# tuneinsight/lattigo

Measured on AMD Instinct MI355X. Metric: ciphertext-mul+relin ops/s, higher is better.
Workload: dtype u64; 1 GPU; BGV logN=15, 12 Q-limbs [55,45x11] + 3 P-limbs [55x3], T=65537: ct x ct MulRelin (tensor + gadget product + ModDown), inputs resident in HBM; batch_per_gpu=256, logN=15, L=12, alpha=3, beta=4, parallelism=1 independent replicas, ciphertext-sharded

## Files before the change

lattigo_amd/csrc/kernels.hip:

```cpp
#include "kernels.h"

#include <atomic>
#include <cstdio>
#include <cstdlib>
#include <type_traits>
#include <mutex>
#include <unordered_map>
#include <vector>

namespace he {

namespace {
struct ProfRec { int id; hipEvent_t e0, e1; double bytes; };
struct ProfState { std::vector<ProfRec> recs; };
std::mutex g_prof_mu;
std::atomic<int> g_prof_active{0};
std::unordered_map<hipStream_t, ProfState> g_prof;
std::vector<hipEvent_t> g_prof_pool;
hipEvent_t prof_event_locked() {
    if (!g_prof_pool.empty()) { hipEvent_t e = g_prof_pool.back(); g_prof_pool.pop_back(); return e; }
    hipEvent_t e;
    (void)hipEventCreate(&e);
    return e;
}
// ... 1315 lines not shown
            const uint64_t qu = ldc(mcw, 0);
            uint64_t r0[16], r1[16], r2[16], r3[16];
            round0(xA);
            __syncthreads();
            rows_lds_xfer_f64<LOGB, 4>(xA, lds, tau, 0, LOGB - 4, true);
            if (AA.e.ext_f64) {
#pragma unroll
                for (int k = 0; k < 16; k++) xB[k] = __longlong_as_double((long long)wB[k]);
            } else {
#pragma unroll
                for (int k = 0; k < 16; k++) xB[k] = u52_to_f64(wB[k]);
            }
            round0(xB);
            __syncthreads();
            MAC_STAMP2(50);
            round1(xA, tau);
            __syncthreads();
            rows_lds_xfer_f64<LOGB, 4>(xB, lds, tau, 0, LOGB - 4, true);
            MAC_STAMP2(51);
            __builtin_amdgcn_sched_barrier(0);
            {
                const uint64_t *pa0 = AA.e.ta0 + meoff(AA.e, ME_TA0, AA.e.ta0_bs, cur.bz, AA.nbatch) + off;
                const uint64_t *pb0 = AA.e.tb0 + meoff(AA.e, ME_TB0, AA.e.tb0_bs, cur.bz, AA.nbatch) + off;
#pragma unroll
                for (int k = 0; k < 16; k++) { r0[k] = pa0[(unsigned)(k * T)]; r1[k] = pb0[(unsigned)(k * T)]; }
            }
            __builtin_amdgcn_sched_barrier(0);
            rows_round16_f64<false>(xA, t2, q, qi);
#pragma unroll
            for (int k = 0; k < 16; k++) xA[k] -= reduce_f64(acc0[k], q, qi);
            __syncthreads();
            MAC_STAMP2(52);
            round1(xB, tau);
            mac_final_xfer<LOGB>(xA, lds, tau, true);
            MAC_STAMP2(53);
            rows_round16_f64<false>(xB, t2, q, qi);
#pragma unroll
            for (int k = 0; k < 16; k++) xB[k] -= reduce_f64(acc1[k], q, qi);
            __builtin_amdgcn_sched_barrier(0);
            {
                const uint64_t *pa1 = AA.e.ta1 + meoff(AA.e, ME_TA1, AA.e.ta1_bs, cur.bz, AA.nbatch) + off;
                const uint64_t *pb1 = AA.e.tb1 + meoff(AA.e, ME_TB1, AA.e.tb1_bs, cur.bz, AA.nbatch) + off;
#pragma unroll
                for (int k = 0; k < 16; k++) { r2[k] = pa1[(unsigned)(k * T)]; r3[k] = pb1[(unsigned)(k * T)]; }
            }
            __builtin_amdgcn_sched_barrier(0);
            __syncthreads();
            MAC_STAMP2(54);
#pragma unroll
            for (int k = 0; k < 16; k++) xA[k] = lds[lds_phys(k * T + tau)];
            __syncthreads();
            mac_final_xfer<LOGB>(xB, lds, tau, true);
            MAC_STAMP2(55);
            auto cvtb = [&](uint64_t (&w)[16], double (&dd)[16]) {
                const uint64_t twoq_u = qu << 1, brc0 = ldc(mcw, 2);
                bool big = false;
#pragma unroll
                for (int k = 0; k < 16; k++) big = big || w[k] >= twoq_u;
                if (__any(big)) {
#pragma unroll
                    for (int k = 0; k < 16; k++) w[k] = bred_add_lazy(w[k], qu, brc0);
                }
#pragma unroll
                for (int k = 0; k < 16; k++) dd[k] = u52_to_f64(w[k]);
            };
            const double tsp = AA.e.tsp[cur.l];
            double u[16], v[16];
            cvtb(r0, u); cvtb(r1, v);
#pragma unroll
            for (int k = 0; k < 16; k++) {
                const double tt = modmul_f64(modmul_f64(u[k], v[k], q, qi), tsp, q, qi) + modmul_f64(xA[k], sp, q, qi);
                stnt(&op0[(unsigned)(k * T)], canon_f64(tt, q, qi));
            }
            __builtin_amdgcn_sched_barrier(0);
            __syncthreads();
            MAC_STAMP2(56);
#pragma unroll
            for (int k = 0; k < 16; k++) xB[k] = lds[lds_phys(k * T + tau)];
            double u2[16], v2[16];
            cvtb(r2, u2); cvtb(r3, v2);
#pragma unroll
            for (int k = 0; k < 16; k++) {
                const double wv = modmul_f64(u[k], v2[k], q, qi) + modmul_f64(u2[k], v[k], q, qi);
                const double tt = modmul_f64(wv, tsp, q, qi) + modmul_f64(xB[k], sp, q, qi);
                stnt(&op1[(unsigned)(k * T)], canon_f64(tt, q, qi));
            }
            MAC_STAMP2(57);
        } else if constexpr (EPI) {
            auto ext_pass = [&](auto cc) __attribute__((always_inline)) {
                const int c = cc;
                unsigned tau_d = threadIdx.x;
                asm volatile("" : "+v"(tau_d));
                const unsigned tau = tau_d, lane = tau & 63u;
                const double *pw = pbuf + wv * 1024u + lane;
                MAC_STAMP2(48 + c * 4 + 0);
                asm volatile("s_waitcnt vmcnt(0)" ::: "memory");
                double x[16];
                if (AA.e.ext_f64) {
#pragma unroll
                    for (int k = 0; k < 16; k++) x[k] = pw[k * 64];
                } else {
#pragma unroll
                    for (int k = 0; k < 16; k++) x[k] = u52_to_f64((uint64_t)__double_as_longlong(pw[k * 64]));
                }
                const uint64_t *nsrc = next_src(A.m.beta + c);
                const bool second = c != 0;
                const size_t off = (size_t)cur.out_limb * A.N + cur.rowoff + tau;
                uint64_t *op = (second ? AA.e.out1 + meoff(AA.e, ME_OUT1, AA.e.out1_bs, cur.bz, AA.nbatch) : AA.e.out0 + meoff(AA.e, ME_OUT0, AA.e.out0_bs, cur.bz, AA.nbatch)) + off;
                const double sp = AA.e.sp[cur.l];
                const uint64_t *mcw = reinterpret_cast<const uint64_t *>(A.mc + cur.mi);
                const uint64_t qu = ldc(mcw, 0);
                const bool tensor = LOGB == 13 && AA.e.tensor != 0;
                const bool addw = !tensor && (second ? AA.e.has_w1 : AA.e.has_w0) != 0;
                double kd0[16], kd1[16];
                MAC_STAMP2(48 + c * 4 + 1);
                constexpr bool prefetch = LOGB == 12;
                const uint64_t *pa0 = nullptr, *pa1 = nullptr, *pb0 = nullptr, *pb1 = nullptr, *wp = nullptr;
                if (tensor) {
                    pa0 = AA.e.ta0 + meoff(AA.e, ME_TA0, AA.e.ta0_bs, cur.bz, AA.nbatch) + off; pa1 = AA.e.ta1 + meoff(AA.e, ME_TA1, AA.e.ta1_bs, cur.bz, AA.nbatch) + off;
                    pb0 = AA.e.tb0 + meoff(AA.e, ME_TB0, AA.e.tb0_bs, cur.bz, AA.nbatch) + off; pb1 = AA.e.tb1 + meoff(AA.e, ME_TB1, AA.e.tb1_bs, cur.bz, AA.nbatch) + off;
                } else if (addw) {
                    wp = (second ? AA.e.w1 + meoff(AA.e, ME_W1, AA.e.w1_bs, cur.bz, AA.nbatch) : AA.e.w0 + meoff(AA.e, ME_W0, AA.e.w0_bs, cur.bz, AA.nbatch)) + off;
                }
                constexpr int NB = 4;
                uint64_t A0[NB], A1[NB], A2[NB], A3[NB];
                if constexpr (prefetch) transform(addw ? 1 : 0, x, tau, lane, nsrc, reinterpret_cast<const double *>(wp), nullptr, kd0, kd1);
                else transform(0, x, tau, lane, nsrc, nullptr, nullptr, kd0, kd1);
#pragma unroll
                for (int k = 0; k < 16; k++) x[k] -= reduce_f64(acc0[k], q, qi);
                mac_final_xfer<LOGB>(x, lds, tau, true);
                __syncthreads();
#pragma unroll
                for (int k = 0; k < 16; k++) x[k] = lds[lds_phys(k * T + tau)];
                MAC_STAMP2(48 + c * 4 + 2);
                if (tensor) {
                    const double tsp = AA.e.tsp[cur.l];
                    const uint64_t twoq_u = qu << 1, brc0 = ldc(mcw, 2);
                    auto cvtb = [&](uint64_t (&w)[NB], double (&dd)[NB]) {
                        bool big = false;
#pragma unroll
                        for (int k = 0; k < NB; k++) big = big || w[k] >= twoq_u;
                        if (__any(big)) {
#pragma unroll
                            for (int k = 0; k < NB; k++) w[k] = bred_add_lazy(w[k], qu, brc0);
                        }
#pragma unroll
                        for (int k = 0; k < NB; k++) dd[k] = u52_to_f64(w[k]);
                    };
                    auto issue = [&](auto hc, uint64_t (&r0)[NB], uint64_t (&r1)[NB], uint64_t (&r2)[NB], uint64_t (&r3)[NB]) {
                        constexpr int h = decltype(hc)::value;
#pragma unroll
                        for (int k = 0; k < NB; k++) { const unsigned e = (unsigned)((NB * h + k) * T); r0[k] = pa0[e]; r1[k] = pb0[e]; }
                        if (second) {
#pragma unroll
                            for (int k = 0; k < NB; k++) { const unsigned e = (unsigned)((NB * h + k) * T); r2[k] = pa1[e]; r3[k] = pb1[e]; }
                        }
                        __builtin_amdgcn_sched_barrier(0);
                    };
                    auto finish = [&](auto hc, uint64_t (&r0)[NB], uint64_t (&r1)[NB], uint64_t (&r2)[NB], uint64_t (&r3)[NB]) {
                        constexpr int h = decltype(hc)::value;
                        double u[NB], v[NB], u2[NB], v2[NB], wv[NB];
                        cvtb(r0, u); cvtb(r1, v);
                        if (second) {
                            cvtb(r2, u2); cvtb(r3, v2);
#pragma unroll
                            for (int k = 0; k < NB; k++) wv[k] = modmul_f64(u[k], v2[k], q, qi) + modmul_f64(u2[k], v[k], q, qi);
                        } else {
#pragma unroll
                            for (int k = 0; k < NB; k++) wv[k] = modmul_f64(u[k], v[k], q, qi);
                        }
#pragma unroll
                        for (int k = 0; k < NB; k++) {
                            const int i = NB * h + k;
                            const double tt = modmul_f64(wv[k], tsp, q, qi) + modmul_f64(x[i], sp, q, qi);
                            stnt(&op[(unsigned)(i * T)], canon_f64(tt, q, qi));
                        }
                        __builtin_amdgcn_sched_barrier(0);
                    };
#define HE_H(n) std::integral_constant<int, n>{}
                    issue(HE_H(0), A0, A1, A2, A3); finish(HE_H(0), A0, A1, A2, A3);
                    issue(HE_H(1), A0, A1, A2, A3); finish(HE_H(1), A0, A1, A2, A3);
                    issue(HE_H(2), A0, A1, A2, A3); finish(HE_H(2), A0, A1, A2, A3);
                    issue(HE_H(3), A0, A1, A2, A3); finish(HE_H(3), A0, A1, A2, A3);
#undef HE_H
                } else if (addw) {
                    uint64_t wv[16];
                    if constexpr (prefetch) {
#pragma unroll
                        for (int k = 0; k < 16; k++) wv[k] = (uint64_t)__double_as_longlong(kd0[k]);
                    } else {
#pragma unroll
                        for (int k = 0; k < 16; k++) wv[k] = ldnt(&wp[(unsigned)(k * T)]);
                    }
#pragma unroll
                    for (int k = 0; k < 16; k++) {
                        const uint64_t v = canon_f64(modmul_f64(x[k], sp, q, qi), q, qi);
                        uint64_t *dp = &op[(unsigned)(k * T)];
                        if constexpr (SCAT) dp = op - (cur.rowoff + tau) + auto_dest((unsigned)(cur.rowoff + tau) + (unsigned)(k * T), AA.e.sc_ginv, AA.e.sc_logN);
                        stnt(dp, cred(wv[k] + v, qu));
                    }
                } else {
#pragma unroll
                    for (int k = 0; k < 16; k++) {
                        uint64_t *dp = &op[(unsigned)(k * T)];
                        if constexpr (SCAT) dp = op - (cur.rowoff + tau) + auto_dest((unsigned)(cur.rowoff + tau) + (unsigned)(k * T), AA.e.sc_ginv, AA.e.sc_logN);
                        stnt(dp, canon_f64(modmul_f64(x[k], sp, q, qi), q, qi));
                    }
                }
                MAC_STAMP2(48 + c * 4 + 3);
#pragma unroll
                for (int k = 0; k < 16; k++) acc0[k] = acc1[k];
            };
            if constexpr (LOGB == 12) {
                ext_pass(std::integral_constant<int, 0>{});
                ext_pass(std::integral_constant<int, 1>{});
            } else {
#pragma unroll 1
                for (int c = 0; c < 2; c++) ext_pass(c);
            }
        }
        const int ol = cur.out_limb;
        uint64_t *o0 = nullptr, *o1 = nullptr;
        unsigned tau_t = threadIdx.x;
        asm volatile("" : "+v"(tau_t));
        const unsigned tau = tau_t;
        if constexpr (!EPI) {
            o0 = (cur.isP ? A.o0P + voff(A.oP0_tab, A.oP0_bs, cur.bz) : A.o0Q + voff(A.oQ0_tab, A.oQ0_bs, cur.bz)) + (size_t)ol * A.N + cur.rowoff + tau;
            o1 = (cur.isP ? A.o1P + voff(A.oP1_tab, A.oP1_bs, cur.bz) : A.o1Q + voff(A.oQ1_tab, A.oQ1_bs, cur.bz)) + (size_t)ol * A.N + cur.rowoff + tau;
        }
        [[maybe_unused]] uint64_t gs_av[16], gs_p0[16], gs_p1[16];
        [[maybe_unused]] const uint64_t *gs_ap = nullptr;
        if constexpr (!EPI && SCAT) {
            __builtin_amdgcn_sched_barrier(0);
            const size_t src = cur.rowoff + tau;
            if (AA.e.has_w0) gs_ap = (cur.isP ? AA.e.w1 + meoff(AA.e, ME_W1, AA.e.w1_bs, cur.bz, AA.nbatch) : AA.e.w0 + meoff(AA.e, ME_W0, AA.e.w0_bs, cur.bz, AA.nbatch)) + (size_t)ol * A.N + src;
            if (gs_ap) {
#pragma unroll
                for (int k = 0; k < 16; k++) gs_av[k] = ldnt(&gs_ap[(unsigned)(k * T)]);
            }
            if (AA.e.gs_accum) {
                const uint64_t *b0p = o0 - src;
#pragma unroll
                for (int k = 0; k < 16; k++) gs_p0[k] = b0p[auto_dest((unsigned)src + (unsigned)(k * T), AA.e.sc_ginv, AA.e.sc_logN)];
            }
            __builtin_amdgcn_sched_barrier(0);
        }
        if constexpr (!EPI) {
            auto to_natural = [&](double (&a)[16]) {
                mac_final_xfer<LOGB>(a, lds, tau, true);
                __syncthreads();
#pragma unroll
                for (int k = 0; k < 16; k++) a[k] = lds[lds_phys(k * T + tau)];
            };
            to_natural(acc0);
            if constexpr (SCAT) {
                const uint64_t qu = ldc(reinterpret_cast<const uint64_t *>(A.mc + cur.mi), 0);
                const size_t src = cur.rowoff + tau;
                uint64_t *b0p = o0 - src;
                const uint64_t *b1p = o1 - src;
                const bool accum = AA.e.gs_accum != 0;
                if (accum) {
#pragma unroll
                    for (int k = 0; k < 16; k++) gs_p1[k] = b1p[auto_dest((unsigned)src + (unsigned)(k * T), AA.e.sc_ginv, AA.e.sc_logN)];
                }
                __builtin_amdgcn_sched_barrier(0);
#pragma unroll
                for (int k = 0; k < 16; k++) {
                    uint64_t v0 = canon_f64(acc0[k], q, qi);
                    if (gs_ap) v0 = cred(v0 + gs_av[k], qu);
                    if (accum) v0 += gs_p0[k];
                    stnt(&b0p[auto_dest((unsigned)src + (unsigned)(k * T), AA.e.sc_ginv, AA.e.sc_logN)], v0);
                }
            }
            __syncthreads();
            to_natural(acc1);
        }
        if constexpr (EPI) {
            (void)o0; (void)o1; (void)ol;
        } else if constexpr (SCAT) {
            const size_t src = cur.rowoff + tau;
            uint64_t *b1p = o1 - src;
            const bool accum = AA.e.gs_accum != 0;
#pragma unroll
            for (int k = 0; k < 16; k++) {
                uint64_t v1 = canon_f64(acc1[k], q, qi);
                if (accum) v1 += gs_p1[k];
                stnt(&b1p[auto_dest((unsigned)src + (unsigned)(k * T), AA.e.sc_ginv, AA.e.sc_logN)], v1);
            }
        } else if constexpr (QF64) {
            double *d0 = reinterpret_cast<double *>(o0), *d1 = reinterpret_cast<double *>(o1);
#pragma unroll
            for (int k = 0; k < 16; k++) {
                stnt(&d0[(unsigned)(k * T)], reduce_f64(acc0[k], q, qi));
                stnt(&d1[(unsigned)(k * T)], reduce_f64(acc1[k], q, qi));
            }
        } else {
#pragma unroll
            for (int k = 0; k < 16; k++) {
                o0[(unsigned)(k * T)] = canon_f64(acc0[k], q, qi);
                o1[(unsigned)(k * T)] = canon_f64(acc1[k], q, qi);
            }
        }
        MAC_STAMP2(60);
        if (!more) break;
        cur = decode(w);
    }
}

static unsigned mac_resident_workgroups(int logb) {
    static const unsigned cus = [] {
        int dev = 0, n = 0;
        if (hipGetDevice(&dev) != hipSuccess || hipDeviceGetAttribute(&n, hipDeviceAttributeMultiprocessorCount, dev) != hipSuccess || n <= 0)
            n = 256;
        return (unsigned)n;
    }();
    return logb >= 13 ? cus : 2u * cus;
}

bool ntt_prod_in_supported(int logN) {
    const int b = ntt_row_bits(logN);
    return b == 12 || b == 13;
}
bool epilogue_scatter_supported(int logN) {
    const int b = ntt_row_bits(logN);
    return b == 12 || b == 13;
}
bool ntt_mac_epilogue_supported(int logN) {
    const int b = ntt_row_bits(logN);
    return b == 12 || b == 13;
}
bool ntt_mac_giant_supported(int logN) {
    const int b = ntt_row_bits(logN);
    return b == 12 || b == 13;
}
hipError_t launch_ntt_mac_f64(const RingDev &r, const NttMacArgs &a, View dec, View own, const double *keyd, View out0Q,
                              View out0P, View out1Q, View out1P, int batch, hipStream_t s, const NttMacEpilogue *epi,
                              const KsScatter *giant) {
    if (a.nlimbs <= 0 || batch <= 0) return hipSuccess;
    if (!r.twd_fwd || !keyd) return hipErrorInvalidValue;
    if (giant && (epi || a.q_out_f64 || !giant->ginv || !ntt_mac_giant_supported(r.logN))) return hipErrorInvalidValue;
    if (dec.tab || (epi && epi->ext.tab) || (a.q_out_f64 && !no_tab({out0Q, out1Q}))) return hipErrorInvalidValue;
    const int b = ntt_row_bits(r.logN), aa = r.logN - b;
    if (epi && !ntt_mac_epilogue_supported(r.logN)) return hipErrorInvalidValue;
    NttMacKArgs A{};
    A.dec = dec.p; A.dec_bs = dec.bstride; A.own = own.p; A.own_bs = own.bstride; A.own_tab = own.tab; A.keyd = keyd;
    A.o0Q = out0Q.p; A.o0P = out0P.p; A.o1Q = out1Q.p; A.o1P = out1P.p;
    A.oQ0_bs = out0Q.bstride; A.oP0_bs = out0P.bstride; A.oQ1_bs = out1Q.bstride; A.oP1_bs = out1P.bstride;
    A.oQ0_tab = out0Q.tab; A.oP0_tab = out0P.tab; A.oQ1_tab = out1Q.tab; A.oP1_tab = out1P.tab;
    A.mc = r.mc; A.twd = r.twd_fwd; A.N = r.N; A.a = aa; A.m = a;
    double mac_bytes = ((double)a.beta * batch + 2.0 * a.beta + 2.0 * batch) * a.nlimbs * (double)r.N * 8.0;
    if (epi) mac_bytes += (2.0 + (epi->tensor ? 4.0 : (epi->has_w0 ? 1.0 : 0.0) + (epi->has_w1 ? 1.0 : 0.0))) * batch * a.nlimbs * (double)r.N * 8.0;
    if (epi || giant || b >= 12) {
        NttMacDmaArgs D;
        D.k = A;
        D.e = MacEpiK{};
        if (epi) {
            D.e.ext = epi->ext.p; D.e.ext_bs = epi->ext.bstride; D.e.ext_f64 = epi->ext_f64 ? 1 : 0;
            D.e.out0 = epi->out0.p; D.e.out0_bs = epi->out0.bstride; D.e.out1 = epi->out1.p; D.e.out1_bs = epi->out1.bstride;
            D.e.has_w0 = epi->has_w0 ? 1 : 0; D.e.has_w1 = epi->has_w1 ? 1 : 0;
            D.e.w0 = epi->w0.p; D.e.w0_bs = epi->w0.bstride; D.e.w1 = epi->w1.p; D.e.w1_bs = epi->w1.bstride;
            D.e.tensor = epi->tensor ? 1 : 0;
            if (epi->scatter_ginv && epi->tensor) return hipErrorInvalidValue;
            D.e.sc_ginv = epi->scatter_ginv; D.e.sc_logN = r.logN;
            D.e.ta0 = epi->ta0.p; D.e.ta0_bs = epi->ta0.bstride; D.e.ta1 = epi->ta1.p; D.e.ta1_bs = epi->ta1.bstride;
            D.e.tb0 = epi->tb0.p; D.e.tb0_bs = epi->tb0.bstride; D.e.tb1 = epi->tb1.p; D.e.tb1_bs = epi->tb1.bstride;
            {
                const View *vs[8] = {&epi->out0, &epi->out1, &epi->w0, &epi->w1, &epi->ta0, &epi->ta1, &epi->tb0, &epi->tb1};
                const size_t *base = nullptr;
                for (const View *v : vs) if (v->tab && (!base || v->tab < base)) base = v->tab;
                D.e.etab = base;
                D.e.etab_rows = 0xFFFFFFFFu;
                for (int i = 0; i < 8 && base; i++) {
                    if (!vs[i]->tab) continue;
                    const size_t d = (size_t)(vs[i]->tab - base);
                    if (d % (size_t)batch != 0 || d / (size_t)batch >= 15) return hipErrorInvalidValue;
                    D.e.etab_rows = (D.e.etab_rows & ~(0xFu << (4 * i))) | ((unsigned)(d / (size_t)batch) << (4 * i));
                }
            }
            for (int i = 0; i < a.nlimbs; i++) { D.e.sp[i] = epi->sp[i]; D.e.tsp[i] = epi->tsp[i]; }
        }
        if (giant) {
            D.e.sc_ginv = giant->ginv; D.e.sc_logN = r.logN;
            D.e.has_w0 = giant->add0.p ? 1 : 0;
            D.e.w0 = giant->add0.p; D.e.w0_bs = giant->add0.bstride; D.e.w1 = giant->add0P.p; D.e.w1_bs = giant->add0P.bstride;
            D.e.gs_accum = giant->accumulate ? 1 : 0;
            const View *vs[2] = {&giant->add0, &giant->add0P};
            const size_t *base = nullptr;
            for (const View *v : vs) if (v->tab && (!base || v->tab < base)) base = v->tab;
            D.e.etab = base;
            D.e.etab_rows = 0xFFFFFFFFu;
            for (int i = 0; i < 2 && base; i++) {
                if (!vs[i]->tab) continue;
                const size_t d = (size_t)(vs[i]->tab - base);
                if (d % (size_t)batch != 0 || d / (size_t)batch >= 15) return hipErrorInvalidValue;
                const int which = i == 0 ? ME_W0 : ME_W1;
                D.e.etab_rows = (D.e.etab_rows & ~(0xFu << (4 * which))) | ((unsigned)(d / (size_t)batch) << (4 * which));
            }
            mac_bytes += ((giant->add0.p ? 1.0 : 0.0) + (giant->accumulate ? 2.0 : 0.0)) * batch * a.nlimbs * (double)r.N * 8.0;
        }
        D.nbatch = (unsigned)batch;
        D.nitems = (unsigned)batch * (unsigned)a.nlimbs * (1u << aa);
        for (int i = 0; i < a.nlimbs; i++)
            D.limb_info[i] = (uint64_t)a.mod[i] | (uint64_t)a.key_limb[i] << 8 | (uint64_t)a.dec_limb[i] << 16 |
                             (uint64_t)a.out_limb[i] << 24 | (uint64_t)a.out_view[i] << 32;
        unsigned G = mac_resident_workgroups(b);
        if (D.nitems <= G) G = D.nitems;
        else {
            const unsigned per = (D.nitems + G - 1) / G;
            G = (D.nitems + per - 1) / per;
            if ((D.nitems & 7u) == 0) G = (G + 7u) & ~7u;
        }
        ProfScope ps(K_NTT_MAC_F64, s, mac_bytes);
        if (epi && D.e.sc_ginv) {
            if (b == 12) hipLaunchKernelGGL((ntt_mac_f64_dma_kernel<12, false, true, true>), dim3(G), dim3(256), 0, s, D);
            else hipLaunchKernelGGL((ntt_mac_f64_dma_kernel<13, false, true, true>), dim3(G), dim3(512), 0, s, D);
        } else if (epi && D.e.tensor && b == 12) {
            hipLaunchKernelGGL((ntt_mac_f64_dma_kernel<12, false, true, false, true>), dim3(G), dim3(256), 0, s, D);
        } else if (epi) {
            if (b == 12) hipLaunchKernelGGL((ntt_mac_f64_dma_kernel<12, false, true>), dim3(G), dim3(256), 0, s, D);
            else hipLaunchKernelGGL((ntt_mac_f64_dma_kernel<13, false, true>), dim3(G), dim3(512), 0, s, D);
        } else if (giant) {
            if (b == 12) hipLaunchKernelGGL((ntt_mac_f64_dma_kernel<12, false, false, true>), dim3(G), dim3(256), 0, s, D);
            else hipLaunchKernelGGL((ntt_mac_f64_dma_kernel<13, false, false, true>), dim3(G), dim3(512), 0, s, D);
        } else if (b == 12) {
            if (a.q_out_f64) hipLaunchKernelGGL((ntt_mac_f64_dma_kernel<12, true>), dim3(G), dim3(256), 0, s, D);
            else hipLaunchKernelGGL((ntt_mac_f64_dma_kernel<12, false>), dim3(G), dim3(256), 0, s, D);
        } else {
            if (a.q_out_f64) hipLaunchKernelGGL((ntt_mac_f64_dma_kernel<13, true>), dim3(G), dim3(512), 0, s, D);
            else hipLaunchKernelGGL((ntt_mac_f64_dma_kernel<13, false>), dim3(G), dim3(512), 0, s, D);
        }
        return hipGetLastError();
    }
    dim3 grid(batch, a.nlimbs, 1u << aa);
    ProfScope ps(K_NTT_MAC_F64, s, mac_bytes);
#define HE_MAC_CASE(B)                                                                                      \
    case B:                                                                                                 \
        if (a.q_out_f64) hipLaunchKernelGGL((ntt_mac_f64_kernel<B, true>), grid, dim3((1 << B) / 16), 0, s, A);  \
        else hipLaunchKernelGGL((ntt_mac_f64_kernel<B, false>), grid, dim3((1 << B) / 16), 0, s, A);             \
        break;
    switch (b) {
        HE_MAC_CASE(4) HE_MAC_CASE(5) HE_MAC_CASE(6) HE_MAC_CASE(7) HE_MAC_CASE(8) HE_MAC_CASE(9) HE_MAC_CASE(10)
        HE_MAC_CASE(11)
        default: return hipErrorInvalidValue;
    }
#undef HE_MAC_CASE
    return hipGetLastError();
}

struct KeyF64Args {
    const uint64_t *key;
    double *keyd;
    const ModConst *mc;
    int N, nlimbs;
    int rowbits;
    uint8_t mod[kMaxLimbs];
};
__global__ void __launch_bounds__(256) key_to_f64_kernel(KeyF64Args A) {
    const int x = blockIdx.x * blockDim.x + threadIdx.x;
    if (x >= A.N) return;
    const int l = blockIdx.y;
    const size_t base = ((size_t)blockIdx.z * A.nlimbs + l) * A.N;
    const ModConst m = A.mc[A.mod[l]];
    size_t dst = (size_t)x;
    if (A.rowbits > 0) {
        const unsigned e = (unsigned)x & ((1u << A.rowbits) - 1u), T = 1u << (A.rowbits - 4);
        dst = (size_t)((unsigned)x - e) + (e & 15u) * T + (e >> 4);
    }
    A.keyd[base + dst] = (m.q >> kF64Bits) == 0 ? (double)imform(A.key[base + x], m.q, m.qinv) : 0.0;
}
hipError_t launch_key_to_f64(const RingDev &r, const uint64_t *key, double *keyd, int nblocks, const uint8_t *limb_mod_host,
                             int nlimbs, hipStream_t s) {
    KeyF64Args A{};
    A.key = key; A.keyd = keyd; A.mc = r.mc; A.N = r.N; A.nlimbs = nlimbs;
    A.rowbits = ntt_row_bits(r.logN) >= 12 ? ntt_row_bits(r.logN) : 0;
    for (int i = 0; i < nlimbs; i++) A.mod[i] = limb_mod_host[i];
    dim3 grid((unsigned)((r.N + 255) / 256), nlimbs, nblocks), block(256);
    hipLaunchKernelGGL(key_to_f64_kernel, grid, block, 0, s, A);
    return hipGetLastError();
}

template <int LOGA, bool INV, bool INNER = false>
__global__ void __launch_bounds__(256) ntt_cols_kernel(NttArgs A) {
    constexpr int R = 1 << LOGA;
    const int cbits = INNER ? A.cb : 0;
    const int N2 = (A.N >> cbits) >> LOGA;
    const int cg = blockIdx.x * blockDim.x + threadIdx.x;
    if (cg >= (A.N >> LOGA)) return;
    const int blk = INNER ? cg >> __builtin_ctz((unsigned)N2) : 0, c = INNER ? cg & (N2 - 1) : cg;
    const int rowtw = INNER ? (1 << cbits) + blk : 1;
    const int y = blockIdx.y;
    const int il = A.tab.in_limb[y], ol = A.tab.out_limb[y], mi = A.tab.mod[y];
    const ModConst mc = A.mc[mi];
    const uint64_t q = mc.q, qinv = mc.qinv, twoq = mc.q << 1;
    const uint64_t *__restrict__ tw = A.tw + (size_t)mi * A.N;
    const size_t e0 = (size_t)blk * ((size_t)N2 << LOGA) + c;
    const uint64_t *__restrict__ src = A.in + voff(A.in_tab, A.in_bs, blockIdx.z) + (size_t)il * A.N + e0;
    uint64_t *__restrict__ dst = A.out + voff(A.out_tab, A.out_bs, blockIdx.z) + (size_t)ol * A.N + e0;

    uint64_t x[R];
#pragma unroll
    for (int r = 0; r < R; r++) x[r] = src[(size_t)r * N2];
    if (!INV && (A.flags & NTT_ADD_SCALAR)) {
        const uint64_t sadd = A.io_s[y];
#pragma unroll
        for (int r = 0; r < R; r++) x[r] += sadd;
    }
    if (A.flags & NTT_REDUCE_INPUT) {
#pragma unroll
        for (int r = 0; r < R; r++) x[r] = bred_add_lazy(x[r], q, mc.brc0);
    }
    if constexpr (!INV) {
        const bool nc = (q >> kNoCorrBits) == 0;
#pragma unroll
        for (int s = 0; s < LOGA; s++) {
            const int d = 1 << (LOGA - 1 - s);
#pragma unroll
            for (int r = 0; r < R; r++) {
                if (r & d) continue;
                if (nc) bfly_fwd_nc(x[r], x[r + d], tw[(rowtw << s) + (r >> (LOGA - s))], q, qinv);
                else bfly_fwd(x[r], x[r + d], tw[(rowtw << s) + (r >> (LOGA - s))], q, twoq, qinv);
            }
        }
    } else {
#pragma unroll
        for (int s = LOGA - 1; s >= 0; s--) {
            const int d = 1 << (LOGA - 1 - s);
#pragma unroll
            for (int r = 0; r < R; r++) {
                if (r & d) continue;
                const uint64_t wv = tw[(rowtw << s) + (r >> (LOGA - s))];
                if (s == 0 && A.scale) {
                    const uint64_t wn = mred(wv, mc.ninv, q, qinv);
                    bfly_inv_scaled(x[r], x[r + d], wn, mc.ninv, q, twoq, qinv);
                } else {
                    bfly_inv(x[r], x[r + d], wv, q, twoq, qinv);
                }
            }
        }
    }
    if (INV && (A.flags & NTT_ADD_SCALAR) && A.scale) {
        const uint64_t sadd = A.io_s[y];
#pragma unroll
        for (int r = 0; r < R; r++) x[r] = cred(x[r] + sadd, q);
    }
#pragma unroll
    for (int r = 0; r < R; r++) dst[(size_t)r * N2] = x[r];
}

static double rows_bytes(dim3 grid, const NttArgs &A, int logb) {
    const double entries = A.epi_tensor ? 2.0 * A.zsplit : (A.nbatch_prof > 0 ? (double)A.nbatch_prof : (double)grid.x);
    double streams = A.tprod ? 4.0 : 2.0;
    if (A.epi) streams += 1.0 + (A.epi_tensor ? 2.0 : (A.epi == 2 || (A.zsplit && A.epi2 == 2)) ? 1.0 : 0.0);
    return entries * grid.y * grid.z * (double)(1u << logb) * 8.0 * streams;
}
template <bool INV, bool NC>
static hipError_t launch_rows_nc(int logb, dim3 grid, const NttArgs &A, hipStream_t s) {
    static const bool no_lean = env_flag("HERING_NO_LEAN_INV_ROWS");
    if constexpr (INV) {
        if (!no_lean && (logb == 12 || logb == 13) && !A.scale) {
            ProfScope ps(K_NTT_ROWS_INV, s, rows_bytes(grid, A, logb));
            if (logb == 12) hipLaunchKernelGGL((ntt_rows_kernel<12, true, false, true>), grid, dim3(256), 0, s, A);
            else hipLaunchKernelGGL((ntt_rows_kernel<13, true, false, true>), grid, dim3(512), 0, s, A);
            return hipGetLastError();
        }
    }
    if constexpr (!INV) {
        if (A.sc_ginv) {
            if ((logb != 12 && logb != 13) || !A.epi) return hipErrorInvalidValue;
            ProfScope ps(K_NTT_ROWS_FWD, s, rows_bytes(grid, A, logb));
            if (logb == 12) hipLaunchKernelGGL((ntt_rows_kernel<12, false, NC, false, true>), grid, dim3(256), 0, s, A);
            else hipLaunchKernelGGL((ntt_rows_kernel<13, false, NC, false, true>), grid, dim3(512), 0, s, A);
            return hipGetLastError();
        }
    }
#define HE_ROWS_CASE(B)                                                                           \
    case B:                                                                                       \
        { ProfScope ps(INV ? K_NTT_ROWS_INV : K_NTT_ROWS_FWD, s, rows_bytes(grid, A, B));                                 \
        hipLaunchKernelGGL((ntt_rows_kernel<B, INV, NC>), grid, dim3((1 << B) / 16), 0, s, A); }   \
        break;
    switch (logb) {
        HE_ROWS_CASE(4) HE_ROWS_CASE(5) HE_ROWS_CASE(6) HE_ROWS_CASE(7) HE_ROWS_CASE(8) HE_ROWS_CASE(9)
        HE_ROWS_CASE(10) HE_ROWS_CASE(11) HE_ROWS_CASE(12) HE_ROWS_CASE(13)
        default: return hipErrorInvalidValue;
    }
#undef HE_ROWS_CASE
    return hipGetLastError();
}
template <bool INV>
static hipError_t launch_rows_f64(int logb, dim3 grid, const NttArgs &A, hipStream_t s) {
    if constexpr (INV) {
        if (A.tprod) {
            if (logb != 12 && logb != 13) return hipErrorInvalidValue;
            ProfScope ps(K_NTT_ROWS_INV_F64, s, rows_bytes(grid, A, logb));
            if (logb == 12) hipLaunchKernelGGL((ntt_rows_f64_kernel<12, true, true>), grid, dim3(256), 0, s, A);
            else hipLaunchKernelGGL((ntt_rows_f64_kernel<13, true, true>), grid, dim3(512), 0, s, A);
            return hipGetLastError();
        }
    }
    if constexpr (!INV) {
        if (A.sc_ginv) {
            if ((logb != 12 && logb != 13) || !A.epi) return hipErrorInvalidValue;
            ProfScope ps(K_NTT_ROWS_FWD_F64, s, rows_bytes(grid, A, logb));
            if (logb == 12) hipLaunchKernelGGL((ntt_rows_f64_kernel<12, false, false, true>), grid, dim3(256), 0, s, A);
            else hipLaunchKernelGGL((ntt_rows_f64_kernel<13, false, false, true>), grid, dim3(512), 0, s, A);
            return hipGetLastError();
        }
    }
#define HE_ROWSF_CASE(B)                                                                          \
    case B:                                                                                       \
        { ProfScope ps(INV ? K_NTT_ROWS_INV_F64 : K_NTT_ROWS_FWD_F64, s, rows_bytes(grid, A, B));                         \
        hipLaunchKernelGGL((ntt_rows_f64_kernel<B, INV>), grid, dim3((1 << B) / 16), 0, s, A); }   \
        break;
    switch (logb) {
        HE_ROWSF_CASE(4) HE_ROWSF_CASE(5) HE_ROWSF_CASE(6) HE_ROWSF_CASE(7) HE_ROWSF_CASE(8) HE_ROWSF_CASE(9)
        HE_ROWSF_CASE(10) HE_ROWSF_CASE(11) HE_ROWSF_CASE(12) HE_ROWSF_CASE(13)
        default: return hipErrorInvalidValue;
    }
#undef HE_ROWSF_CASE
    return hipGetLastError();
}
template <bool INV>
static hipError_t launch_rows(int logb, dim3 grid, const NttArgs &A, const uint8_t *cls, hipStream_t s) {
    if (!cls) return launch_rows_nc<INV, false>(logb, grid, A, s);
    NttArgs P[3] = {A, A, A};
    for (auto &p : P) p.tab.n = 0;
    for (int i = 0; i < A.tab.n; i++) {
        int c = cls[A.tab.mod[i]];
        if (c == 2 && !A.twd) c = 1;
        if (INV && c == 1) c = 0;
        NttArgs &D = P[c];
        D.tab.in_limb[D.tab.n] = A.tab.in_limb[i];
        D.tab.out_limb[D.tab.n] = A.tab.out_limb[i];
        D.tab.mod[D.tab.n] = A.tab.mod[i];
        D.epi_s[D.tab.n] = A.epi_s[i];
        D.io_s[D.tab.n] = A.io_s[i];
        D.epi_ts[D.tab.n] = A.epi_ts[i];
        D.tab.n++;
    }
    hipError_t e = hipSuccess;
    if (P[2].tab.n) {
        const size_t wgs = (size_t)grid.x * P[2].tab.n * grid.z;
        int iters = (!INV || logb > 12 || P[2].tprod) ? 1 : (wgs >= 6144 ? 2 : 1);
        if (iters > (int)grid.x) iters = (int)grid.x;
        P[2].nbatch = (int)grid.x; P[2].iters = iters; P[2].nbatch_prof = (int)grid.x;
        dim3 g2((grid.x + iters - 1) / iters, P[2].tab.n, grid.z);
        e = launch_rows_f64<INV>(logb, g2, P[2], s);
    }
    P[0].tprod = P[1].tprod = 0;
    if (e == hipSuccess && P[1].tab.n) { dim3 g2(grid.x, P[1].tab.n, grid.z); e = launch_rows_nc<INV, true>(logb, g2, P[1], s); }
    if (e == hipSuccess && P[0].tab.n) { dim3 g2(grid.x, P[0].tab.n, grid.z); e = launch_rows_nc<INV, false>(logb, g2, P[0], s); }
    return e;
}
template <bool INV>
static hipError_t launch_cols(int loga, dim3 grid, const NttArgs &A, hipStream_t s) {
#define HE_COLS_CASE(Av)                                                                 \
    case Av:                                                                             \
        { ProfScope ps(INV ? K_NTT_COLS_INV : K_NTT_COLS_FWD, s, 2.0 * A.tab.n * grid.z * (double)A.N * 8.0);                        \
        hipLaunchKernelGGL((ntt_cols_kernel<Av, INV>), grid, dim3(256), 0, s, A); }       \
        break;
    if (A.cb > 0) {
        if (loga != 4) return hipErrorInvalidValue;
        ProfScope ps(INV ? K_NTT_COLS_INV : K_NTT_COLS_FWD, s, 2.0 * A.tab.n * grid.z * (double)A.N * 8.0);
        hipLaunchKernelGGL((ntt_cols_kernel<4, INV, true>), grid, dim3(256), 0, s, A);
        return hipGetLastError();
    }
    switch (loga) {
        HE_COLS_CASE(1) HE_COLS_CASE(2) HE_COLS_CASE(3) HE_COLS_CASE(4) HE_COLS_CASE(5)
        default: return hipErrorInvalidValue;
    }
#undef HE_COLS_CASE
    return hipGetLastError();
}

static void set_epilogue(NttArgs &A, const NttEpilogue &epi, int n) {
    A.epi_y_f64 = epi.y_small_f64 ? 1 : 0;
    A.epi_y_reduce = epi.y_reduce ? 1 : 0;
    A.epi = epi.has_w ? 2 : 1;
    A.epi_y = epi.y.p; A.epi_y_bs = epi.y.bstride; A.epi_y_tab = epi.y.tab;
    A.epi_w = epi.w.p; A.epi_w_bs = epi.w.bstride; A.epi_w_tab = epi.w.tab;
    for (int i = 0; i < n; i++) A.epi_s[i] = epi.s[i];
    A.epi_tensor = epi.tensor ? 1 : 0;
    A.sc_ginv = epi.tensor ? 0u : epi.scatter_ginv;
    A.sc_logN = 0;
    for (int nn = A.N; nn > 1; nn >>= 1) A.sc_logN++;
    if (epi.tensor) {
        A.ta0 = epi.ta0.p; A.ta1 = epi.ta1.p; A.tb0 = epi.tb0.p; A.tb1 = epi.tb1.p;
        A.ta0_bs = epi.ta0.bstride; A.ta1_bs = epi.ta1.bstride; A.tb0_bs = epi.tb0.bstride; A.tb1_bs = epi.tb1.bstride;
        A.ta0_tab = epi.ta0.tab; A.ta1_tab = epi.ta1.tab; A.tb0_tab = epi.tb0.tab; A.tb1_tab = epi.tb1.tab;
        for (int i = 0; i < n; i++) A.epi_ts[i] = epi.ts[i];
    }
    if (epi.zsplit > 0) {
        A.zsplit = epi.zsplit; A.epi2 = epi.has_w2 ? 2 : 1;
        A.out2 = epi.out2.p; A.out2_bs = epi.out2.bstride; A.out2_tab = epi.out2.tab;
        A.epi_y2 = epi.y2.p; A.epi_y2_bs = epi.y2.bstride; A.epi_y2_tab = epi.y2.tab;
        A.epi_w2 = epi.w2.p; A.epi_w2_bs = epi.w2.bstride; A.epi_w2_tab = epi.w2.tab;
    }
}
hipError_t launch_ntt(const RingDev &r, const LimbTab &tab, View in, View out, int batch, bool inverse, int flags,
                      hipStream_t s, const uint64_t *io_scalar, const NttEpilogue *epi) {
    if (tab.n <= 0 || batch <= 0) return hipSuccess;
    const int n = r.logN;
    if (n < 4 || n > kMaxLogN) return hipErrorInvalidValue;
    if (epi && (inverse || epi->zsplit > 0)) return hipErrorInvalidValue;
    const int b = ntt_row_bits(n), a = n - b;
    const int a_out = a > 5 ? a - 4 : a, a_in = a - a_out;
    NttArgs A{};
    A.mc = r.mc;
    A.N = r.N;
    A.a = a;
    A.tab = tab;
    A.epi = 0; A.epi_y = A.epi_w = nullptr; A.epi_y_bs = A.epi_w_bs = 0;
    A.zsplit = 0; A.epi2 = 0; A.out2 = nullptr; A.out2_bs = 0; A.epi_y2 = A.epi_w2 = nullptr; A.epi_y2_bs = A.epi_w2_bs = 0;
    A.epi_y_f64 = 0; A.epi_y_reduce = 0; A.epi_tensor = 0;
    const int sflag = io_scalar ? NTT_ADD_SCALAR : 0;
    for (int i = 0; i < tab.n; i++) A.io_s[i] = io_scalar ? io_scalar[i] : 0;
    dim3 grows(batch, tab.n, 1u << a);
    dim3 gcols((unsigned)(((r.N >> a_out) + 255) / 256), tab.n, batch);
    dim3 gcols_in((unsigned)(((r.N >> (a_in > 0 ? a_in : 1)) + 255) / 256), tab.n, batch);
    hipError_t e;
    if (!inverse) {
// ... 3553 lines not shown
```

Baseline: 43870 ctxt-mul+relin ops/s.

## Add 512-thread radix-8 fused NTT-MAC tensor kernel as default path

Adds a new fused NTT+key-MAC+tensor epilogue kernel for the 4096-row case that uses 512 threads with 8 elements per thread, in place of the existing 256-thread kernel with 16 elements per thread. It does three radix-8 passes through padded LDS, stages per-row twiddles in shared memory and double-buffers digit DMA. It is meant to lower register pressure and raise occupancy or latency hiding in the gadget-product/ModDown stage. The old kernel stays reachable through an environment flag. The cost is more block-wide syncs and LDS traffic per transform.

```diff
diff --git a/lattigo_amd/csrc/kernels.hip b/lattigo_amd/csrc/kernels.hip
--- a/lattigo_amd/csrc/kernels.hip
+++ b/lattigo_amd/csrc/kernels.hip
@@ -1641,6 +1641,323 @@
             }
         }
         MAC_STAMP2(60);
+        if (!more) break;
+        cur = decode(w);
+    }
+}
+
+__device__ __forceinline__ unsigned t8_phys(unsigned e) { return e + (e >> 3); }
+__device__ __forceinline__ void rows_round8_f64(double (&x)[8], const double (&t)[7], double q, double qi) {
+#pragma unroll
+    for (int u = 0; u < 3; u++) {
+        const int d = 1 << (2 - u);
+#pragma unroll
+        for (int k = 0; k < 8; k++) {
+            if (k & d) continue;
+            const double r = modmul_f64(x[k + d], t[(1 << u) - 1 + (k >> (3 - u))], q, qi);
+            const double U = x[k];
+            x[k] = U + r;
+            x[k + d] = U - r;
+        }
+    }
+}
+typedef const NttMacDmaArgs __attribute__((address_space(4))) *t8_args_ptr;
+__device__ __forceinline__ t8_args_ptr t8_launder(t8_args_ptr p) {
+    uintptr_t v = (uintptr_t)p;
+    asm volatile("" : "+s"(v));
+    return (t8_args_ptr)v;
+}
+__global__ void __launch_bounds__(512, 4) ntt_mac_f64_t8_kernel(NttMacDmaArgs AA) {
+    constexpr int N2 = 4096, T = 512;
+    t8_args_ptr P = t8_launder((t8_args_ptr)__builtin_amdgcn_kernarg_segment_ptr());
+    auto meoff8 = [&](int which, size_t bs, size_t z) -> size_t {
+        const unsigned row = (P->e.etab_rows >> (4 * which)) & 0xFu;
+        return (P->e.etab && row != 0xFu) ? (size_t)ldc(reinterpret_cast<const uint64_t *>(P->e.etab), (size_t)row * P->nbatch + z) : z * bs;
+    };
+    __shared__ double lds[N2 + N2 / 8];
+    __shared__ double pbuf[N2];
+    __shared__ double tw2s[64 * 7];
+
+    const unsigned tau = threadIdx.x, lane = tau & 63u;
+    const unsigned wv = (unsigned)__builtin_amdgcn_readfirstlane((int)(tau >> 6));
+    const unsigned G = gridDim.x, g = blockIdx.x;
+    const bool xcd = ((G | P->nitems) & 7u) == 0;
+    const unsigned span = xcd ? P->nitems >> 3 : P->nitems, stride = xcd ? G >> 3 : G;
+    const unsigned first = xcd ? g >> 3 : g, base = xcd ? (g & 7u) * span : 0u;
+    auto item_of = [&](unsigned t) -> unsigned { const unsigned i = first + t * stride; return i < span ? base + i : ~0u; };
+
+    struct Item {
+        size_t bz, rowoff;
+        int ql, rowtw, out_limb, mi, l;
+        bool isP;
+        double q, qi;
+        const double *tw, *kbase;
+    };
+    auto decode = [&](unsigned w) -> Item {
+        Item it;
+        it.bz = w % P->nbatch;
+        const int l = (int)((w / P->nbatch) % (unsigned)P->k.m.nlimbs);
+        const int row = (int)(w / (P->nbatch * (unsigned)P->k.m.nlimbs));
+        const uint64_t info = P->limb_info[l];
+        it.l = l;
+        const int mi = (int)(info & 0xff);
+        it.mi = mi;
+        const uint64_t *mcw = reinterpret_cast<const uint64_t *>(P->k.mc + mi);
+        it.q = (double)ldc(mcw, 0); it.qi = __longlong_as_double((long long)ldc(mcw, 8));
+        it.tw = P->k.twd + (size_t)mi * P->k.N;
+        it.rowtw = (1 << P->k.a) + row;
+        it.rowoff = (size_t)row * N2;
+        it.kbase = P->k.keyd + (size_t)((info >> 8) & 0xff) * P->k.N + it.rowoff;
+        it.ql = (int)((info >> 16) & 0xff);
+        it.out_limb = (int)((info >> 24) & 0xff);
+        it.isP = ((info >> 32) & 0xff) != 0;
+        return it;
+    };
+    auto own_digit = [&](const Item &it, int d) -> bool {
+        return P->k.m.own_alpha > 0 && !it.isP && it.ql >= d * P->k.m.own_alpha && it.ql < (d + 1) * P->k.m.own_alpha;
+    };
+    const int nd = P->k.m.beta + 2;
+    auto digit_src = [&](const Item &it, int d) -> const uint64_t * {
+        if (d >= P->k.m.beta)
+            return P->e.ext + ((size_t)(d - P->k.m.beta) * P->nbatch + it.bz) * P->e.ext_bs + (size_t)it.ql * P->k.N + it.rowoff;
+        return own_digit(it, d) ? P->k.own + voff(P->k.own_tab, P->k.own_bs, it.bz) + (size_t)it.ql * P->k.N + it.rowoff
+                                : P->k.dec + it.bz * P->k.dec_bs + (size_t)d * P->k.m.dec_dstride + (size_t)it.ql * P->k.N + it.rowoff;
+    };
+    const unsigned pw_addr = lds_byte_addr(pbuf) + wv * 4096u;
+    auto dma_digit = [&](const uint64_t *src, unsigned lane) {
+        const uint64_t *gp = src + ((lane >> 5) * T + 64u * wv + 2u * (lane & 31u));
+#pragma unroll
+        for (int j = 0; j < 4; j++) glds16(gp + (size_t)j * 2 * T, pw_addr + (unsigned)j * 1024u);
+    };
+
+    unsigned t = 0;
+    unsigned w = item_of(0);
+    if (w == ~0u) return;
+    Item cur = decode(w);
+    dma_digit(digit_src(cur, 0), lane);
+    for (;;) {
+        P = t8_launder(P);
+        double acc0[8], acc1[8];
+#pragma unroll
+        for (int k = 0; k < 8; k++) { acc0[k] = 0.0; acc1[k] = 0.0; }
+        const double q = cur.q, qi = cur.qi;
+        unsigned tau_w = threadIdx.x;
+        asm volatile("" : "+v"(tau_w));
+        if (tau_w < 448u) {
+            const unsigned tau = tau_w, hi = tau / 7u, idx = tau - hi * 7u, u = 31u - (unsigned)__builtin_clz(idx + 1u), j = idx + 1u - (1u << u);
+            tw2s[tau] = cur.tw[((unsigned)cur.rowtw << (6 + u)) + (hi << u) + j];
+        }
+        bool more = false;
+        auto transform = [&](int nk, double (&x)[8], unsigned tau, unsigned lane, const uint64_t *nsrc, const double *k0p,
+                             const double *k1p, unsigned rs, double (&kk0)[8], double (&kk1)[8]) {
+            double t3[7];
+#pragma unroll
+            for (int u = 0; u < 3; u++)
+#pragma unroll
+                for (int j = 0; j < (1 << u); j++) t3[(1 << u) - 1 + j] = cur.tw[((unsigned)cur.rowtw << (9 + u)) + (tau << u) + j];
+            __builtin_amdgcn_sched_barrier(0);
+            asm volatile("s_waitcnt lgkmcnt(0)" ::: "memory");
+            if (nsrc) dma_digit(nsrc, lane);
+            __builtin_amdgcn_sched_barrier(0);
+            {
+                double t0[7];
+#pragma unroll
+                for (int u = 0; u < 3; u++)
+#pragma unroll
+                    for (int j = 0; j < (1 << u); j++) t0[(1 << u) - 1 + j] = ldcd(cur.tw, (size_t)(((unsigned)cur.rowtw << u) + j));
+                rows_round8_f64(x, t0, q, qi);
+            }
+            __syncthreads();
+#pragma unroll
+            for (int k = 0; k < 8; k++) lds[t8_phys((unsigned)(k * T) + tau)] = x[k];
+            __syncthreads();
+            const unsigned b1 = wv * 512u + lane;
+#pragma unroll
+            for (int k = 0; k < 8; k++) x[k] = lds[t8_phys(b1 + (unsigned)(k * 64))];
+            {
+                double t1[7];
+#pragma unroll
+                for (int u = 0; u < 3; u++)
+#pragma unroll
+                    for (int j = 0; j < (1 << u); j++)
+                        t1[(1 << u) - 1 + j] = ldcd(cur.tw, (size_t)(((unsigned)cur.rowtw << (3 + u)) + (wv << u) + j));
+                rows_round8_f64(x, t1, q, qi);
+            }
+#pragma unroll
+            for (int k = 0; k < 8; k++) lds[t8_phys(b1 + (unsigned)(k * 64))] = x[k];
+            wave_lds_sync();
+            const unsigned b2 = (tau >> 3) * 64u + (tau & 7u);
+#pragma unroll
+            for (int k = 0; k < 8; k++) x[k] = lds[t8_phys(b2 + (unsigned)(k * 8))];
+            {
+                double t2[7];
+                const double *tp = tw2s + (tau >> 3) * 7u;
+#pragma unroll
+                for (int i = 0; i < 7; i++) t2[i] = tp[i];
+                rows_round8_f64(x, t2, q, qi);
+            }
+#pragma unroll
+            for (int k = 0; k < 8; k++) lds[t8_phys(b2 + (unsigned)(k * 8))] = x[k];
+            wave_lds_sync();
+#pragma unroll
+            for (int k = 0; k < 8; k++) x[k] = lds[t8_phys(tau * 8u + (unsigned)k)];
+            __builtin_amdgcn_sched_barrier(0);
+            if (nk >= 1) {
+#pragma unroll
+                for (int k = 0; k < 8; k++) kk0[k] = k0p[(unsigned)k * rs];
+            }
+            __builtin_amdgcn_sched_barrier(0);
+            rows_round8_f64(x, t3, q, qi);
+            __builtin_amdgcn_sched_barrier(0);
+            if (nk >= 2) {
+#pragma unroll
+                for (int k = 0; k < 8; k++) kk1[k] = k1p[(unsigned)k * rs];
+            }
+            __builtin_amdgcn_sched_barrier(0);
+        };
+        auto next_src = [&](int d) -> const uint64_t * {
+            if (d + 1 < nd) return digit_src(cur, d + 1);
+            w = item_of(++t);
+            more = w != ~0u;
+            return more ? digit_src(decode(w), 0) : nullptr;
+        };
+        for (int d = 0; d < P->k.m.beta; d++) {
+            const bool is_own = own_digit(cur, d);
+            unsigned tau_d = threadIdx.x;
+            asm volatile("" : "+v"(tau_d));
+            P = t8_launder(P);
+            const unsigned tau = tau_d, lane = tau & 63u;
+            const double *pw = pbuf + wv * 512u + lane;
+            asm volatile("s_waitcnt vmcnt(0)" ::: "memory");
+            uint64_t xi[8];
+#pragma unroll
+            for (int k = 0; k < 8; k++) xi[k] = (uint64_t)__double_as_longlong(pw[k * 64]);
+            double x[8];
+            if (is_own && P->k.m.own_reduce) {
+#pragma unroll
+                for (int k = 0; k < 8; k++) xi[k] = bred_add_lazy(xi[k], ldc(reinterpret_cast<const uint64_t *>(P->k.mc + cur.mi), 0), ldc(reinterpret_cast<const uint64_t *>(P->k.mc + cur.mi), 2));
+            }
+            if (P->k.m.dec_f64 && !is_own) {
+#pragma unroll
+                for (int k = 0; k < 8; k++) x[k] = __longlong_as_double((long long)xi[k]);
+            } else {
+#pragma unroll
+                for (int k = 0; k < 8; k++) x[k] = u52_to_f64(xi[k]);
+            }
+            const uint64_t *nsrc = next_src(d);
+            const double *k0p = cur.kbase + (size_t)d * P->k.m.key_dstride + ((tau & 1u) * 2048u + (tau >> 1)), *k1p = k0p + P->k.m.key_kstride;
+            double kk0[8], kk1[8];
+            if (!is_own) {
+                transform(2, x, tau, lane, nsrc, k0p, k1p, 256u, kk0, kk1);
+            } else {
+                asm volatile("s_waitcnt lgkmcnt(0)" ::: "memory");
+                if (nsrc) dma_digit(nsrc, lane);
+                __builtin_amdgcn_sched_barrier(0);
+#pragma unroll
+                for (int k = 0; k < 8; k++) kk0[k] = k0p[(unsigned)(k * 256)];
+#pragma unroll
+                for (int k = 0; k < 8; k++) kk1[k] = k1p[(unsigned)(k * 256)];
+                __builtin_amdgcn_sched_barrier(0);
+                __syncthreads();
+#pragma unroll
+                for (int k = 0; k < 8; k++) lds[t8_phys((unsigned)(k * T) + tau)] = x[k];
+                __syncthreads();
+#pragma unroll
+                for (int k = 0; k < 8; k++) x[k] = lds[t8_phys(tau * 8u + (unsigned)k)];
+            }
+#pragma unroll
+            for (int k = 0; k < 8; k++) acc0[k] += modmul_f64(x[k], kk0[k], q, qi);
+#pragma unroll
+            for (int k = 0; k < 8; k++) acc1[k] += modmul_f64(x[k], kk1[k], q, qi);
+        }
+        double tu[8], tv[8];
+        auto ext_pass = [&](auto cc) __attribute__((always_inline)) {
+            constexpr bool second = decltype(cc)::value != 0;
+            unsigned tau_d = threadIdx.x;
+            asm volatile("" : "+v"(tau_d));
+            P = t8_launder(P);
+            const unsigned tau = tau_d, lane = tau & 63u;
+            const double *pw = pbuf + wv * 512u + lane;
+            asm volatile("s_waitcnt vmcnt(0)" ::: "memory");
+            double x[8];
+            if (P->e.ext_f64) {
+#pragma unroll
+                for (int k = 0; k < 8; k++) x[k] = pw[k * 64];
+            } else {
+#pragma unroll
+                for (int k = 0; k < 8; k++) x[k] = u52_to_f64((uint64_t)__double_as_longlong(pw[k * 64]));
+            }
+            const uint64_t *nsrc = next_src(P->k.m.beta + (second ? 1 : 0));
+            const size_t off = (size_t)cur.out_limb * P->k.N + cur.rowoff + tau;
+            uint64_t *op = (second ? P->e.out1 + meoff8(ME_OUT1, P->e.out1_bs, cur.bz)
+                                   : P->e.out0 + meoff8(ME_OUT0, P->e.out0_bs, cur.bz)) + off;
+            const double sp = P->e.sp[cur.l], tsp = P->e.tsp[cur.l];
+            const uint64_t *mcw = reinterpret_cast<const uint64_t *>(P->k.mc + cur.mi);
+            const uint64_t qu = ldc(mcw, 0);
+            [[maybe_unused]] double d0[8], d1[8];
+            if constexpr (!second) {
+                const uint64_t *pa0 = P->e.ta0 + meoff8(ME_TA0, P->e.ta0_bs, cur.bz) + off;
+                const uint64_t *pb0 = P->e.tb0 + meoff8(ME_TB0, P->e.tb0_bs, cur.bz) + off;
+                transform(2, x, tau, lane, nsrc, reinterpret_cast<const double *>(pa0), reinterpret_cast<const double *>(pb0), (unsigned)T, d0, d1);
+            } else {
+                transform(0, x, tau, lane, nsrc, nullptr, nullptr, 0u, d0, d1);
+            }
+#pragma unroll
+            for (int k = 0; k < 8; k++) x[k] -= reduce_f64(acc0[k], q, qi);
+            [[maybe_unused]] uint64_t r2[8], r3[8];
+            if constexpr (second) {
+                const uint64_t *pa1 = P->e.ta1 + meoff8(ME_TA1, P->e.ta1_bs, cur.bz) + off;
+                const uint64_t *pb1 = P->e.tb1 + meoff8(ME_TB1, P->e.tb1_bs, cur.bz) + off;
+                __builtin_amdgcn_sched_barrier(0);
+#pragma unroll
+                for (int k = 0; k < 8; k++) { r2[k] = pa1[(unsigned)(k * T)]; r3[k] = pb1[(unsigned)(k * T)]; }
+                __builtin_amdgcn_sched_barrier(0);
+            }
+#pragma unroll
+            for (int k = 0; k < 8; k++) lds[t8_phys(tau * 8u + (unsigned)k)] = x[k];
+            __syncthreads();
+#pragma unroll
+            for (int k = 0; k < 8; k++) x[k] = lds[t8_phys((unsigned)(k * T) + tau)];
+            auto cvtb = [&](uint64_t (&w)[8], double (&dd)[8]) {
+                const uint64_t twoq_u = qu << 1, brc0 = ldc(mcw, 2);
+                bool big = false;
+#pragma unroll
+                for (int k = 0; k < 8; k++) big = big || w[k] >= twoq_u;
+                if (__any(big)) {
+#pragma unroll
+                    for (int k = 0; k < 8; k++) w[k] = bred_add_lazy(w[k], qu, brc0);
+                }
+#pragma unroll
+                for (int k = 0; k < 8; k++) dd[k] = u52_to_f64(w[k]);
+            };
+            if constexpr (!second) {
+                uint64_t r0[8], r1[8];
+#pragma unroll
+                for (int k = 0; k < 8; k++) { r0[k] = (uint64_t)__double_as_longlong(d0[k]); r1[k] = (uint64_t)__double_as_longlong(d1[k]); }
+                cvtb(r0, tu); cvtb(r1, tv);
+            }
+            double (&u)[8] = tu, (&v)[8] = tv;
+            if constexpr (second) {
+                double u2[8], v2[8];
+                cvtb(r2, u2); cvtb(r3, v2);
+#pragma unroll
+                for (int k = 0; k < 8; k++) {
+                    const double cr = modmul_f64(u[k], v2[k], q, qi) + modmul_f64(u2[k], v[k], q, qi);
+                    const double tt = modmul_f64(cr, tsp, q, qi) + modmul_f64(x[k], sp, q, qi);
+                    stnt(&op[(unsigned)(k * T)], canon_f64(tt, q, qi));
+                }
+            } else {
+#pragma unroll
+                for (int k = 0; k < 8; k++) {
+                    const double tt = modmul_f64(modmul_f64(u[k], v[k], q, qi), tsp, q, qi) + modmul_f64(x[k], sp, q, qi);
+                    stnt(&op[(unsigned)(k * T)], canon_f64(tt, q, qi));
+                }
+            }
+#pragma unroll
+            for (int k = 0; k < 8; k++) acc0[k] = acc1[k];
+        };
+        ext_pass(std::integral_constant<int, 0>{});
+        ext_pass(std::integral_constant<int, 1>{});
         if (!more) break;
         cur = decode(w);
     }
@@ -1754,7 +2071,9 @@
             if (b == 12) hipLaunchKernelGGL((ntt_mac_f64_dma_kernel<12, false, true, true>), dim3(G), dim3(256), 0, s, D);
             else hipLaunchKernelGGL((ntt_mac_f64_dma_kernel<13, false, true, true>), dim3(G), dim3(512), 0, s, D);
         } else if (epi && D.e.tensor && b == 12) {
-            hipLaunchKernelGGL((ntt_mac_f64_dma_kernel<12, false, true, false, true>), dim3(G), dim3(256), 0, s, D);
+            static const bool t16 = env_flag("HERING_MAC_T16");
+            if (t16) hipLaunchKernelGGL((ntt_mac_f64_dma_kernel<12, false, true, false, true>), dim3(G), dim3(256), 0, s, D);
+            else hipLaunchKernelGGL(ntt_mac_f64_t8_kernel, dim3(G), dim3(512), 0, s, D);
         } else if (epi) {
             if (b == 12) hipLaunchKernelGGL((ntt_mac_f64_dma_kernel<12, false, true>), dim3(G), dim3(256), 0, s, D);
             else hipLaunchKernelGGL((ntt_mac_f64_dma_kernel<13, false, true>), dim3(G), dim3(512), 0, s, D);
```

Result: no change. 43940 ctxt-mul+relin ops/s (median of 6 runs) (+0.1%).
